# Dale-M/opendht

Measured on AMD Instinct MI355X. Metric: queries/sec, k=8 XOR-NN over 16M 160-bit IDs; % HBM roofline at 1/2/4/8 GPUs, higher is better.
Workload: dtype u32; 1 GPU; cfg2 batched k-NN: 65536 targets x 16777216 ids (2^24), k=8; n_ids=16777216, n_targets=65536, k=8, algo=batch, route=broadcast, ids_per_gpu=16777216, targets_per_gpu=65536, parallelism=id-range shards x1, inflight=3

## Files before the change

### opendht_amd/__init__.py

```python
import ctypes
import os

import numpy as np

__all__ = ["Context", "DhtGpuError", "NONE", "MAX_K", "lib", "LIB_PATH", "id_words"]

LIB_PATH = os.environ.get("DHTGPU_LIB") or os.path.join(os.path.dirname(os.path.abspath(__file__)), "libdhtgpu.so")
NONE = 0xFFFFFFFF
MAX_K = 32
EINVAL, ENOMEM, EDEVICE, ENOIDS, EUNSORTED, ERANGE = -1, -2, -3, -4, -5, -6

_u8p = ctypes.POINTER(ctypes.c_uint8)
_u32p = ctypes.POINTER(ctypes.c_uint32)
_u64p = ctypes.POINTER(ctypes.c_uint64)
_vp = ctypes.c_void_p
_lib = None


class DhtGpuError(RuntimeError):
    def __init__(self, code, what=""):
        msg = _lib.dhtgpu_strerror(code).decode() if _lib is not None else str(code)
        super().__init__(f"libdhtgpu: {what}: {msg} ({code})")
        self.code = code

# ... 167 lines not shown
    def set_global_indices(self, on):
        _check(lib().dhtgpu_set_global_indices(self._h, int(bool(on))), "set_global_indices")

    def set_sub_handles(self, on):
        _check(lib().dhtgpu_set_sub_handles(self._h, int(bool(on))), "set_sub_handles")

    def sub_handles_active(self, q, k):
        return bool(lib().dhtgpu_sub_handles_active(self._h, q, k))

    def handles_to_indices_dev(self, handles_ptr, m, out_ptr, idx_base=0, stream=None):
        _check(lib().dhtgpu_handles_to_indices_dev(self._h, handles_ptr, m, out_ptr, idx_base, stream),
               "handles_to_indices_dev")

    def select_prefix_dev(self, planes_ptr, stride, n, pbits, pval, out_planes_ptr, out_stride, out_gidx_ptr=None,
                          stream=None):
        cnt = ctypes.c_uint64()
        _check(lib().dhtgpu_select_prefix_dev(self._h, planes_ptr, stride, n, pbits, pval, out_planes_ptr, out_stride,
                                              out_gidx_ptr, ctypes.byref(cnt), stream), "select_prefix_dev")
        return cnt.value

    @property
    def num_ids(self):
        return int(lib().dhtgpu_num_ids(self._h))

    def get_ids(self, first=0, n=None):
        if n is None:
            n = self.num_ids - first
        out = np.empty((n, 20), dtype=np.uint8)
        _check(lib().dhtgpu_get_ids(self._h, first, n, _p(out, _u8p)), "get_ids")
        return out

    def ids_dev(self):
        p, s = _vp(), ctypes.c_uint64()
        _check(lib().dhtgpu_ids_dev(self._h, ctypes.byref(p), ctypes.byref(s)), "ids_dev")
        return p.value, s.value

    def topk(self, targets, k=8):
        t = _ids(targets, "targets")
        q = t.shape[0]
        out = np.empty((q, k), dtype=np.uint32)
        cnt = np.empty(q, dtype=np.uint32)
        _check(lib().dhtgpu_topk(self._h, _p(t, _u8p), q, k, _p(out, _u32p), _p(cnt, _u32p)), "topk")
        return out, cnt

    def index_topk(self, targets, k=8):
        t = _ids(targets, "targets")
        q = t.shape[0]
        out = np.empty((q, k), dtype=np.uint32)
        cnt = np.empty(q, dtype=np.uint32)
        _check(lib().dhtgpu_index_topk(self._h, _p(t, _u8p), q, k, _p(out, _u32p), _p(cnt, _u32p)), "index_topk")
        return out, cnt

    def index_build(self, stream=None):
        _check(lib().dhtgpu_index_build(self._h, stream), "index_build")

    def index_build_timed(self, stream=None):
        ms = (ctypes.c_float * 4)()
        _check(lib().dhtgpu_index_build_timed(self._h, stream, ms), "index_build_timed")
        return tuple(ms)

    def index_topk_dev(self, t_planes_ptr, t_stride, q, k, out_idx_ptr=None, out_cnt_ptr=None, out_rec_ptr=None,
                       idx_base=0, stream=None):
        _check(lib().dhtgpu_index_topk_dev(self._h, t_planes_ptr, t_stride, q, k, out_idx_ptr, out_cnt_ptr,
                                           out_rec_ptr, idx_base, stream), "index_topk_dev")

    def batch_topk(self, targets, k=8):
        t = _ids(targets, "targets")
        q = t.shape[0]
        out = np.empty((q, k), dtype=np.uint32)
        cnt = np.empty(q, dtype=np.uint32)
        _check(lib().dhtgpu_batch_topk(self._h, _p(t, _u8p), q, k, _p(out, _u32p), _p(cnt, _u32p)), "batch_topk")
        return out, cnt

    def batch_topk_dev(self, t_planes_ptr, t_stride, q, k, out_idx_ptr=None, out_cnt_ptr=None, out_rec_ptr=None,
                       idx_base=0, stream=None):
        _check(lib().dhtgpu_batch_topk_dev(self._h, t_planes_ptr, t_stride, q, k, out_idx_ptr, out_cnt_ptr,
                                           out_rec_ptr, idx_base, stream), "batch_topk_dev")

    def batch_topk_timed(self, t_planes_ptr, t_stride, q, k, out_idx_ptr, out_cnt_ptr, stream=None):
        ms = (ctypes.c_float * 4)()
        st = (ctypes.c_uint32 * 4)()
        _check(lib().dhtgpu_batch_topk_timed(self._h, t_planes_ptr, t_stride, q, k, out_idx_ptr, out_cnt_ptr,
                                             stream, ms, st), "batch_topk_timed")
        return tuple(ms), int(st[0]), int(st[1]), int(st[2])

    def batch_events(self, events):
        arr = (_vp * 8)(*[e.cuda_event for e in events])
        _check(lib().dhtgpu_batch_events(self._h, arr), "batch_events")

    def tie_words_dev(self, rec_ptr, q, k, idx_base, ties_ptr, tie_cap, row_base, out_words_ptr, stream=None):
        _check(lib().dhtgpu_tie_words_dev(self._h, rec_ptr, q, k, idx_base, ties_ptr, tie_cap, row_base,
                                          out_words_ptr, stream), "tie_words_dev")

    def topk_dev(self, t_planes_ptr, t_stride, q, k, out_idx_ptr=None, out_cnt_ptr=None, out_rec_ptr=None,
                 idx_base=0, stream=None):
        _check(lib().dhtgpu_topk_dev(self._h, t_planes_ptr, t_stride, q, k, out_idx_ptr, out_cnt_ptr,
                                     out_rec_ptr, idx_base, stream), "topk_dev")

    def find_closest(self, firsts, bucket_off, node_ids, good, targets, count=8):
        firsts = _ids(firsts, "firsts") if len(firsts) else np.zeros((0, 20), np.uint8)
        off = np.ascontiguousarray(bucket_off, dtype=np.uint32)
        nodes = _ids(node_ids, "node_ids") if len(node_ids) else np.zeros((1, 20), np.uint8)
        good = np.ascontiguousarray(good, dtype=np.uint8) if len(good) else np.zeros(1, np.uint8)
        t = _ids(targets, "targets")
        q = t.shape[0]
        out = np.empty((q, count), dtype=np.uint32)
        cnt = np.empty(q, dtype=np.uint32)
        _check(lib().dhtgpu_find_closest(self._h, firsts.shape[0], _p(firsts, _u8p), _p(off, _u32p),
                                         _p(nodes, _u8p), _p(good, _u8p), _p(t, _u8p), q, count,
                                         _p(out, _u32p), _p(cnt, _u32p)), "find_closest")
        return out, cnt

    def buffer_nodes(self, node_tail, af, targets, cand):
        t = _ids(targets, "targets")
        q = t.shape[0]
        cand = np.ascontiguousarray(cand, dtype=np.uint32).reshape(q, -1)
        alen = 4 if af == 4 else 16
        tail = np.ascontiguousarray(node_tail, dtype=np.uint8).reshape(-1, alen + 2)
        rec = 20 + alen + 2
        out = np.zeros((q, 8 * rec), dtype=np.uint8)
        ln = np.zeros(q, dtype=np.uint32)
        _check(lib().dhtgpu_buffer_nodes(self._h, _p(tail, _u8p), af, _p(t, _u8p), q, _p(cand, _u32p),
                                         cand.shape[1], _p(out, _u8p), _p(ln, _u32p)), "buffer_nodes")
        return out, ln

    def deserialize_nodes(self, af, myid, blobs, from_af, from_addr):
        alen = 4 if af == 4 else 16
        m = len(blobs)
        off = np.zeros(m + 1, dtype=np.uint64)
        for i, b in enumerate(blobs):
            off[i + 1] = off[i] + len(b)
        blob = np.frombuffer(b"".join(bytes(b) for b in blobs) or b"\0", dtype=np.uint8).copy()
        fa = np.ascontiguousarray(from_af, dtype=np.uint8).reshape(m) if m else np.zeros(1, np.uint8)
        fad = np.ascontiguousarray(from_addr, dtype=np.uint8).reshape(m, 16) if m else np.zeros((1, 16), np.uint8)
        cap = max(1, int(off[-1]) // (20 + alen + 2))
        ids = np.zeros((cap, 20), np.uint8)
        tail = np.zeros((cap, alen + 2), np.uint8)
        st = np.zeros(cap, np.uint8)
        ms = np.zeros(max(m, 1), np.uint8)
        nrec = ctypes.c_uint32()
        my = np.ascontiguousarray(myid, dtype=np.uint8).reshape(20)
        _check(lib().dhtgpu_deserialize_nodes(self._h, af, _p(my, _u8p), _p(blob, _u8p), _p(off, _u64p), m,
                                              _p(fa, _u8p), _p(fad, _u8p), _p(ids, _u8p), _p(tail, _u8p),
                                              _p(st, _u8p), _p(ms, _u8p), ctypes.byref(nrec)), "deserialize_nodes")
        r = nrec.value
        return ids[:r], tail[:r], st[:r], ms[:m]

    def net_prepare(self, dead=None, table_seed=0x5EED):
        d = None
        if dead is not None:
            d = np.ascontiguousarray(dead, dtype=np.uint8)
            if d.shape[0] != self.num_ids:
                raise ValueError("dead mask must have one byte per id")
        _check(lib().dhtgpu_net_prepare(self._h, _p(d, _u8p) if d is not None else None, table_seed), "net_prepare")

    def set_search_alpha(self, alpha):
        _check(lib().dhtgpu_set_search_alpha(self._h, int(alpha)), "set_search_alpha")
        self._alpha = int(alpha)

    def search_batch(self, targets, searchers, max_rounds=64, alpha=None):
        t = _ids(targets, "targets")
        q = t.shape[0]
        sr = np.ascontiguousarray(searchers, dtype=np.uint32).reshape(q)
        idx = np.empty((q, 64), np.uint32)
        fl = np.empty((q, 64), np.uint8)
        ln, rd, qs = (np.empty(q, np.uint32) for _ in range(3))
# ... 119 lines not shown
```

### opendht_amd/csrc/batch.hip

```cpp
#include "scan_dev.h"
#include <hip/hip_ext.h>

#include <mutex>

#include <algorithm>
#include <cmath>
#include <cstdlib>
#include <cstdio>
#include <string>
#include <vector>

namespace dhtgpu {
namespace {

constexpr int kF1Threads = 256;
constexpr int kF3Threads = 256;
constexpr uint32_t kF3Cap = 4096;
constexpr uint32_t kF3Per = kF3Cap / kF3Threads;
constexpr uint32_t kMaxLm = 19;
constexpr uint32_t kMaxSubBits = 11;
constexpr uint32_t kMaxQ = 1u << 22;
constexpr uint32_t kTieSlots = 8;
constexpr uint32_t kSets = 8;
constexpr uint32_t kCtrStride = 64;
// ... 648 lines not shown
                const uint32_t j0 = sb + tid4;
                const uint32_t v4[4] = {ring[r].x, ring[r].y, ring[r].z, ring[r].w};
                const uint32_t rem = hi - sb;
                uint32_t bw[4];
#pragma unroll
                for (uint32_t f = 0; f < 4; ++f) bw[f] = bm[__builtin_amdgcn_ubfe(v4[f], pre_off + 5, lm5) - wbase];
                bool sv[4];
                uint64_t bal[4], any = 0;
#pragma unroll
                for (uint32_t f = 0; f < 4; ++f) {
                    const uint32_t pre = __builtin_amdgcn_ubfe(v4[f], pre_off, a.Lm);
                    sv[f] = __builtin_amdgcn_ubfe(bw[f], pre, 1) != 0 && tid4 + f < rem;
                    bal[f] = __builtin_amdgcn_ballot_w64(sv[f]);
                    any |= bal[f];
                }
                if (any) {
                    const uint32_t l0 = (uint32_t)__ffsll((long long)any) - 1, l1 = 63u - (uint32_t)__clzll(any);
                    const uint32_t mylo = sv[0] ? v4[0] : sv[1] ? v4[1] : sv[2] ? v4[2] : v4[3];
                    const uint32_t myhi = sv[3] ? v4[3] : sv[2] ? v4[2] : sv[1] ? v4[1] : v4[0];
                    const uint32_t plo = top_bits((uint32_t)__builtin_amdgcn_readlane((int)mylo, (int)l0), a.b1);
                    const uint32_t phi = top_bits((uint32_t)__builtin_amdgcn_readlane((int)myhi, (int)l1), a.b1);
                    for (uint32_t p = plo; p <= phi; ++p) {
                        uint64_t bp[4];
                        uint32_t tot = 0;
#pragma unroll
                        for (uint32_t f = 0; f < 4; ++f) {
                            bp[f] = plo == phi ? bal[f] : bal[f] & __builtin_amdgcn_ballot_w64(top_bits(v4[f], a.b1) == p);
                            tot += (uint32_t)__popcll(bp[f]);
                        }
                        if (!tot) continue;
                        const uint32_t pl = p - p_first;
                        const bool glob = (p == p_first && sh_first) || (p == p_last && sh_last) || pl >= kDirParts;
                        uint32_t base = 0;
                        if (lane == 0) base = glob ? atomicAdd(pc + p, tot) : atomicAdd(cnt + pl, tot);
                        uint32_t pos = __builtin_amdgcn_readfirstlane(base);
#pragma unroll
                        for (uint32_t f = 0; f < 4; ++f) {
                            if ((bp[f] >> lane) & 1ull) {
                                const uint32_t at = __builtin_amdgcn_mbcnt_hi(
                                    (uint32_t)(bp[f] >> 32), __builtin_amdgcn_mbcnt_lo((uint32_t)bp[f], pos));
                                if (at < a.pcap) pb[(uint64_t)p * a.pcap + at] = make_uint2(v4[f], j0 + f);
                            }
                            pos += (uint32_t)__popcll(bp[f]);
                        }
                    }
                }
            }
            ring[r] = f2_load1<NT>(rs, lo, sb + kF2Ring * kF2Sub, lim);
        }
    }
    sync_lds();
    F2_STAMP(2);
    const uint32_t nown = min(p_last - p_first + 1u, kDirParts);
    for (uint32_t i = threadIdx.x; i < nown; i += kF2Threads) {
        const uint32_t p = p_first + i;
        if (!((p == p_first && sh_first) || (p == p_last && sh_last))) pc[p] = cnt[i];
    }
    (void)misc;
    F2_STAMP(5);
}

__device__ __forceinline__ bool id_less(uint32_t da, uint32_t ia, uint32_t db, uint32_t ib,
                                        const uint32_t* __restrict__ planes, uint64_t stride, const uint32_t* t) {
    if (da != db) return da < db;
    if (ia == ib) return false;
    uint32_t wa[DHT_W], wb[DHT_W];
    load_id(planes, stride, ia, wa);
    load_id(planes, stride, ib, wb);
    return xor_less_from(wa, ia, wb, ib, t, 1);
}

__device__ __forceinline__ uint32_t map_out(uint32_t x, const uint32_t* __restrict__ gidx, uint32_t base) {
    return gidx ? gidx[x] : x + base;
}


__device__ __forceinline__ void load_target(const uint32_t* __restrict__ tp, uint64_t ts, uint32_t qi, uint32_t* t) {
#pragma unroll
    for (int j = 0; j < DHT_W; ++j) t[j] = __builtin_amdgcn_readfirstlane(tp[(uint64_t)j * ts + qi]);
}

constexpr uint32_t kLaneMax = 256;

__host__ __device__ inline uint32_t f3_words(uint32_t nsub) {
    return (nsub + 1 + 17 + kF3Threads + 1 + 2 + 1) & ~1u;
}

struct RecOut {
    uint32_t* out;
    const uint32_t* planes;
    uint64_t stride;
    const uint32_t* gidx;
    uint32_t base;
    uint32_t w0_direct;
    uint32_t w0_shift, w0_pre;
};

__device__ __forceinline__ void rec_place(const RecOut& o, const uint32_t* __restrict__ planes, const uint32_t* gidx,
                                          uint32_t base, uint32_t k, uint32_t qi, uint32_t r, uint32_t x, uint32_t w0,
                                          bool w0_ok, uint32_t w1) {
    uint32_t* ro = o.out + ((uint64_t)qi * k + r) * 3;
    if (x == DHT_NONE) {
        ro[0] = DHT_NONE;
        ro[1] = DHT_NONE;
        ro[2] = DHT_NONE;
        return;
    }
    const uint32_t cl = gidx ? gidx[x] : x + base;
    ro[0] = w0_ok ? w0 : planes[x];
    ro[1] = w1;
    ro[2] = o.gidx ? o.gidx[cl] : cl + o.base;
}

struct F3Args {
    const uint2* pbuf; uint32_t* pcount; uint32_t pcap;
    const uint2* tbuf; uint32_t* tcount; uint32_t tcap;
    const uint32_t* tspill;
    uint32_t Lm, b1, Lq;
    uint32_t* bitmap; uint32_t nwords;
    const uint32_t* planes; uint64_t stride; uint64_t n;
    const uint32_t* tp; uint64_t ts; uint32_t k;
    const uint32_t* gidx; uint32_t base;
    uint32_t* out_idx; uint32_t* out_cnt;
    uint32_t* ctr; uint32_t* fb_list;
    uint8_t* fb_sub;
    uint32_t* pstat;
    uint4* tie_hdr;
    uint2* tie_cand;
    uint32_t* tie_cnt;
    const SubDesc* subs; uint32_t np_sub;
    uint32_t dbg;
    unsigned long long* stamps;
    uint32_t cap;
    RecOut rec;
    uint32_t Lmin;
    uint32_t nsets;
};

__device__ __forceinline__ void level_range(const uint32_t* sofs, uint32_t sq, uint32_t Lq, uint32_t Lmin, uint32_t want,
                                            uint32_t& lo, uint32_t& hi) {
    uint32_t L = Lq + 1;
    do {
        --L;
        const uint32_t sh_l = Lq - L;
        lo = sofs[(sq >> sh_l) << sh_l];
        hi = sofs[((sq >> sh_l) + 1) << sh_l];
    } while (hi - lo < want && L > Lmin);
}

__device__ __forceinline__ bool key2_less(uint32_t da, uint32_t a1, uint32_t ia, uint32_t db, uint32_t b1, uint32_t ib,
                                          const uint32_t* __restrict__ planes, uint64_t stride, const uint32_t* t) {
    if (da != db) return da < db;
    if (a1 != b1) return a1 < b1;
    return id_less(da, ia, db, ib, planes, stride, t);
}

__device__ __forceinline__ uint32_t wave_rank64(uint32_t md, uint32_t m1, uint32_t mm, uint32_t lane, bool* tie) {
    uint32_t rank = 0, eq = 0;
    for (uint32_t o = 0; o < mm; ++o) {
        const uint32_t xd = (uint32_t)__builtin_amdgcn_readlane((int)md, (int)o);
        const uint32_t x1 = (uint32_t)__builtin_amdgcn_readlane((int)m1, (int)o);
        rank += (uint32_t)(xd < md) | ((uint32_t)(xd == md) & (uint32_t)(x1 < m1));
        eq |= (uint32_t)(xd == md) & (uint32_t)(x1 == m1) & (uint32_t)(o != lane);
    }
    *tie = eq != 0;
    return rank;
}

// ... 26 lines not shown
}

__device__ void wave_rank_answer(const F3Args& a, uint2 me, uint32_t mm, uint32_t qi, uint32_t t0, uint32_t want,
                                 uint32_t lane) {
    const uint32_t w1 = a.planes[a.stride + (lane < mm ? me.y : 0u)];
    uint32_t t[DHT_W];
    load_target(a.tp, a.ts, qi, t);
    wave_rank_loaded(a, me, mm, qi, t0, want, lane, w1, t);
}

__device__ void f3_wave_answer(const F3Args& a, const uint2* S, uint32_t lo, uint32_t hi, uint32_t qi,
                               uint32_t t0, uint32_t want, uint32_t lane) {
    const uint32_t mm = hi - lo;
    if (mm <= 64) {
        wave_rank_answer(a, S[lo + (lane < mm ? lane : 0u)], mm, qi, t0, want, lane);
        return;
    }
    uint32_t t[DHT_W];
    load_target(a.tp, a.ts, qi, t);
    uint32_t* orow = a.out_idx + (uint64_t)qi * a.k;
    {
        uint32_t ed = DHT_NONE, e1 = DHT_NONE, ei = DHT_NONE, cnt = 0;
        for (uint32_t c = lo; c < hi; c += 64) {
            const bool v = c + lane < hi;
            const uint2 x = v ? S[c + lane] : make_uint2(0u, DHT_NONE);
            const uint32_t xd = x.x ^ t0, xi = x.y;
            const uint32_t x1 = v ? a.planes[a.stride + xi] ^ t[1] : DHT_NONE;
            uint32_t wd = cnt == want ? __builtin_amdgcn_readlane((int)ed, want - 1) : DHT_NONE;
            uint32_t w1 = cnt == want ? __builtin_amdgcn_readlane((int)e1, want - 1) : DHT_NONE;
            uint32_t wi = cnt == want ? __builtin_amdgcn_readlane((int)ei, want - 1) : DHT_NONE;
            uint64_t cm = __ballot(v && (cnt < want || key2_less(xd, x1, xi, wd, w1, wi, a.planes, a.stride, t)));
            while (cm) {
                const uint32_t l = (uint32_t)__ffsll((long long)cm) - 1;
                cm &= cm - 1;
                const uint32_t cd = __builtin_amdgcn_readlane((int)xd, l), c1 = __builtin_amdgcn_readlane((int)x1, l);
                const uint32_t ci = __builtin_amdgcn_readlane((int)xi, l);
                if (cnt == want && !key2_less(cd, c1, ci, wd, w1, wi, a.planes, a.stride, t)) continue;
                const bool closer = lane < cnt && key2_less(ed, e1, ei, cd, c1, ci, a.planes, a.stride, t);
                const uint32_t pos = (uint32_t)__popcll(__ballot(closer));
                const uint32_t ud = __shfl_up(ed, 1), u1 = __shfl_up(e1, 1), ui = __shfl_up(ei, 1);
                if (lane == pos) { ed = cd; e1 = c1; ei = ci; }
                else if (lane > pos) { ed = ud; e1 = u1; ei = ui; }
                cnt = cnt + 1 < want ? cnt + 1 : want;
                wd = cnt == want ? __builtin_amdgcn_readlane((int)ed, want - 1) : DHT_NONE;
                w1 = cnt == want ? __builtin_amdgcn_readlane((int)e1, want - 1) : DHT_NONE;
                wi = cnt == want ? __builtin_amdgcn_readlane((int)ei, want - 1) : DHT_NONE;
            }
        }
        if (a.rec.out) {
            if (lane < a.k)
                rec_place(a.rec, a.planes, a.gidx, a.base, a.k, qi, lane, lane < want ? ei : DHT_NONE, ed ^ t0,
                          a.rec.w0_direct, e1 ^ t[1]);
            return;
        }
        if (lane < want) orow[lane] = map_out(ei, a.gidx, a.base);
    }
    if (lane >= want && lane < a.k) orow[lane] = DHT_NONE;
    if (lane == 0) a.out_cnt[qi] = want;
}

template <int K, int CTRL>
__device__ __forceinline__ void f3_merge(uint32_t (&key)[K], uint32_t& lmin) {
    uint32_t b[K];
#pragma unroll
    for (int r = 0; r < K; ++r) b[r] = (uint32_t)__builtin_amdgcn_mov_dpp((int)key[K - 1 - r], CTRL, 0xF, 0xF, true);
    lmin = min(lmin, (uint32_t)__builtin_amdgcn_mov_dpp((int)lmin, CTRL, 0xF, 0xF, true));
#pragma unroll
    for (int r = 0; r < K; ++r) {
        lmin = min(lmin, max(key[r], b[r]));
        key[r] = min(key[r], b[r]);
    }
#pragma unroll
    for (int d = K / 2; d >= 1; d >>= 1) {
#pragma unroll
        for (int r = 0; r < K; ++r) {
            if (r & d) continue;
            const uint32_t x = min(key[r], key[r + d]), y = max(key[r], key[r + d]);
            key[r] = x;
            key[r + d] = y;
        }
    }
}

#define F3_STAMP(i) \
    do { if (Diag && (a.dbg & 256) && threadIdx.x == 0) a.stamps[(uint64_t)blockIdx.x * 16 + (i)] = __builtin_amdgcn_s_memrealtime(); } while (0)

template <int K, bool Diag, bool Exact, bool Subs>
__global__ __launch_bounds__(kF3Threads) void k_f3_answer(F3Args a) {
    extern __shared__ uint32_t sh[];
    const uint32_t p = blockIdx.x, np = gridDim.x;
    const uint32_t sub = p / a.np_sub, pl = p - sub * a.np_sub;
    if (Subs && a.np_sub != np) {
        const SubDesc d = a.subs[sub];
        a.planes = d.planes;
        a.stride = d.stride;
        a.gidx = d.gidx;
        a.base = d.base;
    }
    F3_STAMP(0);
    const uint32_t nsub = 1u << (a.Lq - a.b1);
    uint32_t* sofs = sh;
    uint32_t* wsum = sofs + nsub + 1;
    uint32_t* slow = wsum + 17;
    uint32_t* ntie = slow + kF3Threads + 1;
    uint2* S = reinterpret_cast<uint2*>(sh + f3_words(nsub));
    uint2* T = S + a.cap;
    for (uint32_t i = pl + a.np_sub * threadIdx.x; i < a.nwords; i += a.np_sub * kF3Threads)
        a.bitmap[sub * a.nwords + i] = 0;
    for (uint32_t i = threadIdx.x; i <= nsub; i += kF3Threads) sofs[i] = 0;
    if (threadIdx.x == 0) ntie[0] = ntie[1] = 0;
    static_assert(kF3Cap / kSets == 2 * kF3Threads && kF3Per == 2 * kSets, "gather layout");
    uint32_t ms[kSets];
#pragma unroll
    for (uint32_t x = 0; x < kSets; ++x) ms[x] = a.pcount[x * np + p];
    const uint32_t mt0 = a.tcount[p * kCtrStride];
    const uint2* tsrc = a.tbuf + (uint64_t)p * a.tcap;
    const uint2 tfirst = tsrc[threadIdx.x < a.tcap ? threadIdx.x : 0u];
    uint2 e[kF3Per];
    const uint2* pb = a.pbuf + (uint64_t)p * a.nsets * a.pcap;
#pragma unroll
    for (uint32_t u = 0; u < kF3Per; ++u) e[u] = make_uint2(0u, 0u);
    const uint32_t mt = mt0 < a.tcap ? mt0 : a.tcap;
    if (p == 0) {
        const uint32_t nsp = a.ctr[kSpill];
        if (nsp) {
            if (threadIdx.x == 0) ntie[2] = atomicAdd(a.ctr, nsp);
            sync_lds();
            for (uint32_t j = threadIdx.x; j < nsp; j += kF3Threads) {
                a.fb_list[ntie[2] + j] = a.tspill[j];
                a.fb_sub[ntie[2] + j] = 255;
            }
        }
    }
    sync_lds();
    uint32_t soff[kSets + 1];
    bool over = false;
    soff[0] = 0;
#pragma unroll
    for (uint32_t x = 0; x < kSets; ++x) {
        over = over || ms[x] > a.pcap;
        soff[x + 1] = soff[x] + (ms[x] < a.pcap ? ms[x] : a.pcap);
    }
    const uint32_t m = soff[kSets];
    if (threadIdx.x < kSets) a.pcount[threadIdx.x * np + p] = 0;
    if (threadIdx.x == 0) {
        a.pstat[p] = m;
        a.tcount[p * kCtrStride] = 0;
        if (p == 0) a.ctr[kSpill] = 0;
    }
    if (mt == 0) return;
    F3_STAMP(1);
    const uint32_t lane = lane_id(), wv = threadIdx.x >> 6;
    constexpr uint32_t NWV = kF3Threads / 64;
    if (m > a.cap || over) {
        if (threadIdx.x == 0) ntie[2] = atomicAdd(a.ctr, mt);
        sync_lds();
        for (uint32_t j = threadIdx.x; j < mt; j += kF3Threads) {
            a.fb_list[ntie[2] + j] = tsrc[j].y;
            a.fb_sub[ntie[2] + j] = (uint8_t)sub;
        }
        return;
    }
    const uint32_t smask = nsub - 1u;
    uint32_t rk[kF3Per];
    const uint32_t sq_sh = 32 - a.Lq;
    uint32_t valid = 0;
    {
#pragma unroll
        for (uint32_t u = 0; u < kF3Per; ++u) {
            const uint32_t j = u * kF3Threads + threadIdx.x;
            uint32_t x = 0, base = 0;
#pragma unroll
            for (uint32_t y = 1; y < kSets; ++y)
                if (j >= soff[y]) { x = y; base = soff[y]; }
            if (j < m) e[u] = pb[x * a.pcap + j - base];
            valid |= (uint32_t)(j < m) << u;
        }
    }
#pragma unroll
    for (uint32_t u = 0; u < kF3Per; ++u) {
        rk[u] = DHT_NONE;
        if ((valid >> u) & 1u) rk[u] = atomicAdd(sofs + __builtin_amdgcn_ubfe(e[u].x, sq_sh, a.Lq - a.b1), 1u);
    }
    sync_lds();
    F3_STAMP(2);
    scan_lds<kF3Threads>(sofs, nsub, wsum);
    if (threadIdx.x == 0) sofs[nsub] = m;
    sync_lds();
#pragma unroll
    for (uint32_t u = 0; u < kF3Per; ++u)
        if (rk[u] != DHT_NONE) S[sofs[__builtin_amdgcn_ubfe(e[u].x, sq_sh, a.Lq - a.b1)] + rk[u]] = e[u];
    F3_STAMP(3);
    const uint32_t want = Exact ? (uint32_t)K : (a.n < a.k ? (uint32_t)a.n : a.k);
    const bool full_row = Exact && ((uintptr_t)a.out_idx & 15) == 0;
    for (uint32_t t0i = 0; t0i < mt; t0i += kF3Threads) {
        const uint32_t mtr = mt - t0i < kF3Threads ? mt - t0i : kF3Threads;
        if (threadIdx.x < mtr) T[threadIdx.x] = t0i ? tsrc[t0i + threadIdx.x] : tfirst;
        if (threadIdx.x == 0) slow[kF3Threads] = 0;
        sync_lds();
        if (t0i == 0) F3_STAMP(4);
        const uint32_t G = a.Lmin >= 12 ? (mtr <= kF3Threads / 4 ? 4u : mtr <= kF3Threads / 2 ? 2u : 1u) : 1u;
        const uint32_t slot = G == 4 ? threadIdx.x >> 2 : G == 2 ? threadIdx.x >> 1 : lane * NWV + wv;
        const uint32_t gj = threadIdx.x & (G - 1);
        uint32_t tq = 0, tt0 = 0, tlo = 0, thi = 0;
        bool tinl = false;
        if (slot < mtr) {
            const uint2 te = T[slot];
            const uint32_t t0 = te.x, qi = te.y;
            uint32_t lo = 0, hi = 0;
            level_range(sofs, top_bits(t0, a.Lq) & smask, a.Lq, a.Lmin, want, lo, hi);
            const uint32_t mm = hi - lo;
            if (t0i == 0) F3_STAMP(8);
            if (mm < want) {
                if (gj == 0) {
                    const uint32_t at = atomicAdd(a.ctr, 1u);
                    a.fb_list[at] = qi;
                    a.fb_sub[at] = (uint8_t)sub;
                }
            } else if (mm > kLaneMax || a.Lm == 0) {
                if (gj == 0) {
                    slow[atomicAdd(slow + kF3Threads, 1u)] = slot;
                    atomicAdd(ntie + 1, 1u);
                }
            } else {
                uint32_t dk[K], ok[K];
                uint32_t rmin = DHT_NONE;
                if (a.Lmin >= 12) {
                    uint32_t key[K];
#pragma unroll
                    for (int r = 0; r < K; ++r) key[r] = DHT_NONE;
                    uint32_t lmin = DHT_NONE;
                    uint32_t o = lo + gj;
                    uint32_t nxt = S[o < hi ? o : lo].x;
                    for (; o < hi; o += G) {
                        const uint32_t c = ((nxt ^ t0) << 12) | o;
                        nxt = S[o + G < hi ? o + G : o].x;
                        lmin = min(lmin, max(c, key[K - 1]));
#pragma unroll
                        for (int r = K - 1; r > 0; --r) key[r] = med3_u32(key[r - 1], key[r], c);
                        key[0] = min(key[0], c);
                    }
                    if (t0i == 0) F3_STAMP(9);
                    if (G >= 2) f3_merge<K, 0xB1>(key, lmin);
                    if (G == 4) f3_merge<K, 0x4E>(key, lmin);
#pragma unroll
                    for (int r = 0; r < K; ++r) {
                        dk[r] = key[r] == DHT_NONE ? DHT_NONE : key[r] >> 12;
                        ok[r] = key[r] & 0xFFFu;
                    }
                    rmin = lmin == DHT_NONE ? DHT_NONE : lmin >> 12;
                } else {
#pragma unroll
                    for (int r = 0; r < K; ++r) { dk[r] = DHT_NONE; ok[r] = DHT_NONE; }
                    uint32_t nxt = S[lo].x;
                    for (uint32_t o = lo; o < hi; ++o) {
                        const uint32_t d = nxt ^ t0;
                        nxt = S[o + 1 < hi ? o + 1 : o].x;
                        const bool ins = d < dk[K - 1];
                        rmin = min(rmin, ins ? dk[K - 1] : d);
                        if (ins) {
#pragma unroll
                            for (int r = K - 1; r > 0; --r) {
                                const bool up = d < dk[r - 1];
                                const bool here = d < dk[r];
                                ok[r] = up ? ok[r - 1] : (here ? o : ok[r]);
                                dk[r] = up ? dk[r - 1] : (here ? d : dk[r]);
                            }
                            if (d < dk[0]) { dk[0] = d; ok[0] = o; }
                        }
                    }
                }
                if (t0i == 0) F3_STAMP(10);
                bool tie = rmin == dk[want - 1];
#pragma unroll
                for (int r = 0; r + 1 < K; ++r) tie = tie || ((uint32_t)r + 1 <= want && dk[r] == dk[r + 1]);
                if (tie && !Subs) {
                    if (gj == 0) {
                        tinl = true;
                        tq = qi;
                        tt0 = t0;
                        tlo = lo;
                        thi = hi;
                        atomicAdd(ntie + 1, 1u);
                    }
                } else if (tie) {
                    uint32_t tsl = kTieSlots;
                    {
                        const uint64_t want_slot = __ballot(gj == 0 && mm <= 64), leaders = __ballot(gj == 0);
                        const uint32_t first = (uint32_t)__ffsll((long long)leaders) - 1;
                        uint32_t base = 0;
                        if (lane == first) {
                            atomicAdd(ntie + 1, (uint32_t)__popcll(leaders));
                            if (want_slot) base = atomicAdd(ntie, (uint32_t)__popcll(want_slot));
                        }
                        base = (uint32_t)__builtin_amdgcn_readlane((int)base, (int)first);
                        const uint32_t leader = lane & ~(G - 1);
                        if (mm <= 64) tsl = base + (uint32_t)__popcll(want_slot & ((1ull << leader) - 1ull));
                    }
                    if (tsl < kTieSlots) {
                        const uint32_t g = p * kTieSlots + tsl;
                        uint2* dst = a.tie_cand + (uint64_t)g * 64;
                        for (uint32_t o = gj; o < mm; o += G) dst[o] = S[lo + o];
                        if (gj == 0) a.tie_hdr[g] = make_uint4(qi, t0, mm, 0u);
                    } else if (gj == 0) {
                        slow[atomicAdd(slow + kF3Threads, 1u)] = slot;
                    }
                } else if (gj == 0 || (K == 8 && a.rec.out && full_row && G > 1 && ((uintptr_t)a.rec.out & 15) == 0)) {
                    uint32_t* orow = a.out_idx + (uint64_t)qi * a.k;
                    uint32_t res[K];
                    if (a.rec.out) {
                        uint32_t w0[K], w1[K], gi[K];
#pragma unroll
                        for (int r = 0; r < K; ++r) {
                            const uint2 e = S[(uint32_t)r < want && ok[r] < a.cap ? ok[r] : 0u];
                            res[r] = e.y;
                            w0[r] = e.x;
                        }
#pragma unroll
                        for (int r = 0; r < K; ++r) {
                            if (!a.rec.w0_direct)
                                w0[r] = a.rec.w0_shift ? ((a.rec.w0_pre | (Subs ? sub : 0u)) << (32 - a.rec.w0_shift)) |
                                                             (w0[r] >> a.rec.w0_shift)
                                                       : a.planes[res[r]];
                            w1[r] = a.planes[a.stride + res[r]];
                            res[r] = map_out(res[r], a.gidx, a.base);
                        }
#pragma unroll
                        for (int r = 0; r < K; ++r) gi[r] = a.rec.gidx ? a.rec.gidx[res[r]] : res[r] + a.rec.base;
                        uint32_t* ro = a.rec.out + (uint64_t)qi * a.k * 3;
                        if (full_row && ((uintptr_t)a.rec.out & 15) == 0) {
                            uint32_t wds[3 * K];
#pragma unroll
                            for (int r = 0; r < K; ++r) {
                                wds[3 * r] = w0[r];
                                wds[3 * r + 1] = w1[r];
                                wds[3 * r + 2] = gi[r];
                            }
                            if (K == 8 && G > 1) {
                                auto put = [&](uint32_t c, uint32_t c_lo, uint32_t c_hi) {
                                    uint32_t x[4];
#pragma unroll
                                    for (int i = 0; i < 4; ++i) {
                                        x[i] = 0u;
#pragma unroll
                                        for (uint32_t cc = 0; cc < 6; ++cc)
                                            if (cc >= c_lo && cc < c_hi) x[i] = c == cc ? wds[(4 * cc + i) % (3 * K)] : x[i];
                                    }
                                    *reinterpret_cast<uint4*>(ro + 4 * c) = make_uint4(x[0], x[1], x[2], x[3]);
                                };
                                put(gj, 0u, 4u);
                                if (gj + G < 6) put(gj + G, 2u, 6u);
                                if (gj + 2 * G < 6) put(gj + 2 * G, 4u, 6u);
                            } else {
#pragma unroll
                                for (int r = 0; r < 3 * K; r += 4)
                                    *reinterpret_cast<uint4*>(ro + r) = make_uint4(wds[r], wds[r + 1], wds[r + 2], wds[r + 3]);
                            }
                        } else {
#pragma unroll
                            for (int r = 0; r < K; ++r) {
// ... 16 lines not shown
                        }
#pragma unroll
                        for (int r = 0; r < K; r += 4)
                            *reinterpret_cast<uint4*>(orow + r) = make_uint4(res[r], res[r + 1], res[r + 2], res[r + 3]);
                        a.out_cnt[qi] = want;
                    } else {
#pragma unroll
                        for (int r = 0; r < K; ++r) res[r] = (uint32_t)r < want ? S[ok[r] < a.cap ? ok[r] : 0u].y : 0u;
                        if (a.gidx) {
#pragma unroll
                            for (int r = 0; r < K; ++r) res[r] = a.gidx[res[r]];
                        } else {
#pragma unroll
                            for (int r = 0; r < K; ++r) res[r] += a.base;
                        }
#pragma unroll
                        for (int r = 0; r < K; ++r)
                            if ((uint32_t)r < a.k) orow[r] = (uint32_t)r < want ? res[r] : DHT_NONE;
                        a.out_cnt[qi] = want;
                    }
                }
            }
        }
        if (!Subs) {
            uint64_t tb = __ballot(tinl);
            while (tb) {
                const int L0 = __ffsll((long long)tb) - 1;
                tb &= tb - 1;
                const uint32_t lo0 = (uint32_t)__builtin_amdgcn_readlane((int)tlo, L0);
                const uint32_t mm0 = (uint32_t)__builtin_amdgcn_readlane((int)thi, L0) - lo0;
                const uint32_t q0 = (uint32_t)__builtin_amdgcn_readlane((int)tq, L0);
                const uint32_t t00 = (uint32_t)__builtin_amdgcn_readlane((int)tt0, L0);
                if (mm0 > 64 || !tb) {
                    f3_wave_answer(a, S, lo0, lo0 + mm0, q0, t00, want, lane);
                    continue;
                }
                const int L1 = __ffsll((long long)tb) - 1;
                const uint32_t lo1 = (uint32_t)__builtin_amdgcn_readlane((int)tlo, L1);
                const uint32_t mm1 = (uint32_t)__builtin_amdgcn_readlane((int)thi, L1) - lo1;
                if (mm1 > 64) {
                    f3_wave_answer(a, S, lo0, lo0 + mm0, q0, t00, want, lane);
                    continue;
                }
                tb &= tb - 1;
                const uint32_t q1 = (uint32_t)__builtin_amdgcn_readlane((int)tq, L1);
                const uint32_t t01 = (uint32_t)__builtin_amdgcn_readlane((int)tt0, L1);
                const uint2 c0 = S[lo0 + (lane < mm0 ? lane : 0u)], c1 = S[lo1 + (lane < mm1 ? lane : 0u)];
                const uint32_t w10 = a.planes[a.stride + (lane < mm0 ? c0.y : 0u)];
                const uint32_t w11 = a.planes[a.stride + (lane < mm1 ? c1.y : 0u)];
                uint32_t tw0[DHT_W], tw1[DHT_W];
                load_target(a.tp, a.ts, q0, tw0);
                load_target(a.tp, a.ts, q1, tw1);
                wave_rank_loaded(a, c0, mm0, q0, t00, want, lane, w10, tw0);
                wave_rank_loaded(a, c1, mm1, q1, t01, want, lane, w11, tw1);
            }
        }
        if (Diag && (a.dbg & 256) && t0i == 0) {
            if (lane == 0) a.stamps[2ull * 8192 * 16 + (uint64_t)blockIdx.x * 16 + wv] = __builtin_amdgcn_s_memrealtime();
        }
        sync_lds();
        if (t0i == 0) F3_STAMP(5);
        if (Diag && (a.dbg & 256) && threadIdx.x == 0 && t0i == 0) {
            a.stamps[(uint64_t)blockIdx.x * 16 + 11] = __builtin_amdgcn_s_memrealtime();
            a.stamps[(uint64_t)blockIdx.x * 16 + 13] = mt;
            a.stamps[(uint64_t)blockIdx.x * 16 + 12] =
                (__builtin_amdgcn_s_getreg((31 << 11) | 4) >> 8 & 0xFFu) | (__builtin_amdgcn_s_getreg((31 << 11) | 20) & 0xFu) << 8;
            a.stamps[(uint64_t)blockIdx.x * 16 + 14] = ntie[0];
        }
        const uint32_t ns = slow[kF3Threads];
        for (uint32_t i = wv; i < ns; i += NWV) {
            const uint2 te = T[slow[i]];
            const uint32_t t0 = __builtin_amdgcn_readfirstlane(te.x);
            const uint32_t qi = __builtin_amdgcn_readfirstlane(te.y);
            uint32_t lo = 0, hi = 0;
            level_range(sofs, top_bits(t0, a.Lq) & smask, a.Lq, a.Lmin, want, lo, hi);
            f3_wave_answer(a, S, __builtin_amdgcn_readfirstlane(lo), __builtin_amdgcn_readfirstlane(hi), qi, t0, want,
                           lane);
        }
        if (ns || t0i + kF3Threads < mt) sync_lds();
        if (t0i == 0) F3_STAMP(6);
    }
    sync_lds();
    if (threadIdx.x == 0 && ntie[1]) atomicAdd(a.ctr + 2, ntie[1]);
    if (threadIdx.x == 0 && ntie[0]) a.tie_cnt[p] = ntie[0] < kTieSlots ? ntie[0] : kTieSlots;
    F3_STAMP(7);
}

constexpr uint32_t kF4Threads = scan::WAVES * 64;
constexpr uint32_t kFbGroup = scan::WAVES * kScanTargets;
constexpr uint32_t kFbBlocks = 256;
constexpr uint32_t kFbCands = 256;
constexpr uint32_t kFbSingle = 64;

struct FbArgs {
    uint32_t* rec;
    uint32_t* done;
    uint32_t nfb;
    uint32_t np_ties;
    uint32_t* hint;
};

__device__ __forceinline__ uint32_t ld_sc1(const uint32_t* p) {
    return __hip_atomic_load(p, __ATOMIC_RELAXED, __HIP_MEMORY_SCOPE_AGENT);
}

__device__ __forceinline__ uint32_t wave_min_u32(uint32_t x) {
#pragma unroll
    for (int o = 32; o >= 1; o >>= 1) x = min(x, (uint32_t)__shfl_xor((int)x, o));
    return x;
}

__device__ void fb_merge(const F3Args& a, const FbArgs& f, uint32_t g, uint32_t S, uint32_t cnt, uint32_t* lds,
                         uint32_t gsize = kFbGroup) {
    const uint32_t lane = lane_id(), wv = threadIdx.x >> 6;
    const uint32_t k = a.k, nt = cnt - g * gsize < gsize ? cnt - g * gsize : gsize;
    uint32_t* buf = lds + wv * 2 * kFbCands;
    for (uint32_t j = wv; j < nt; j += scan::WAVES) {
        const uint32_t qr = __builtin_amdgcn_readfirstlane(a.fb_list[g * gsize + j]);
        uint32_t t[DHT_W];
        load_target(a.tp, a.ts, qr, t);
        for (uint32_t c = lane; c < S * k; c += 64) {
            const uint32_t l = c / k, r = c - l * k;
            const uint32_t* src = f.rec + ((((uint64_t)g * S + l) * kFbGroup + j) * k + r) * 6;
            const uint32_t w0 = ld_sc1(src), ix = ld_sc1(src + 5);
            buf[2 * c] = ix == DHT_NONE ? DHT_NONE : w0 ^ t[0];
            buf[2 * c + 1] = ix;
        }
        __builtin_amdgcn_fence(__ATOMIC_RELEASE, "wavefront");
        __builtin_amdgcn_wave_barrier();
        __builtin_amdgcn_fence(__ATOMIC_ACQUIRE, "wavefront");
        uint32_t p = 0, hd = DHT_NONE, hi = DHT_NONE;
        if (lane < S) {
            hd = buf[2 * lane * k];
            hi = buf[2 * lane * k + 1];
        }
        uint32_t* orow = a.out_idx + (uint64_t)qr * k;
        uint32_t r = 0;
        for (; r < k; ++r) {
            const bool valid = hi != DHT_NONE;
            const uint32_t m = wave_min_u32(valid ? hd : DHT_NONE);
            const uint64_t cand = __ballot(valid && hd == m);
            if (!cand) break;
            uint32_t win = (uint32_t)__ffsll((long long)cand) - 1;
            if (__popcll(cand) > 1) {
                uint64_t rest = cand & (cand - 1);
                while (rest) {
                    const uint32_t l2 = (uint32_t)__ffsll((long long)rest) - 1;
                    rest &= rest - 1;
                    const uint32_t ib = __builtin_amdgcn_readlane((int)hi, (int)win);
                    const uint32_t i2 = __builtin_amdgcn_readlane((int)hi, (int)l2);
                    if (id_less(m, i2, m, ib, a.planes, a.stride, t)) win = l2;
                }
            }
            const uint32_t wi = __builtin_amdgcn_readlane((int)hi, (int)win);
            if (lane == 0) {
                if (a.rec.out)
                    rec_place(a.rec, a.planes, a.gidx, a.base, k, qr, r, wi, m ^ t[0], true, a.planes[a.stride + wi]);
                else
                    orow[r] = map_out(wi, a.gidx, a.base);
            }
            if (lane == win) {
                ++p;
                hd = p < k ? buf[2 * (lane * k + p)] : DHT_NONE;
                hi = p < k ? buf[2 * (lane * k + p) + 1] : DHT_NONE;
            }
        }
// ... 1339 lines not shown
```

Measured before the change: 2.065 billion queries/s.

## Resolve first-word XOR ties in-block via LDS twin hash table

Adds an LDS hash table built during the F3 answer kernel that detects candidate IDs sharing the same first 32-bit word (twins). It records up to 16 such candidates with their second word, so tied top-k rows in the first target batch can be resolved inline instead of being sent to the slower tie/fallback path. This adds atomicCAS hashing work, extra global loads and LDS header space to every block, and only applies in restricted cases (no subs, no record output, first tile).

```diff
diff --git a/opendht_amd/__init__.py b/opendht_amd/__init__.py
--- a/opendht_amd/__init__.py
+++ b/opendht_amd/__init__.py
@@ -273,6 +273,7 @@
         st = (ctypes.c_uint32 * 4)()
         _check(lib().dhtgpu_batch_topk_timed(self._h, t_planes_ptr, t_stride, q, k, out_idx_ptr, out_cnt_ptr,
                                              stream, ms, st), "batch_topk_timed")
+        self.last_batch_stats = tuple(int(x) for x in st)
         return tuple(ms), int(st[0]), int(st[1]), int(st[2])
 
     def batch_events(self, events):
diff --git a/opendht_amd/csrc/batch.hip b/opendht_amd/csrc/batch.hip
--- a/opendht_amd/csrc/batch.hip
+++ b/opendht_amd/csrc/batch.hip
@@ -754,8 +754,22 @@
 
 constexpr uint32_t kLaneMax = 256;
 
+constexpr uint32_t kTwinProbes = 16;
+constexpr uint32_t kTwinCap = 16;
+constexpr uint32_t kTwinWords = 8;
+constexpr uint32_t kTwinMul0 = 0x9E3779B1u, kTwinMul1 = 0x85EBCA6Bu;
+constexpr uint32_t kTwinMinTable = 512;
+constexpr uint32_t kTwinHdr = 4 + kTwinWords + 3 * kTwinCap;
+
+__device__ __forceinline__ uint32_t twin_slot(uint32_t w, uint32_t r, uint32_t tsz, uint32_t hsh) {
+    uint32_t s = (w * kTwinMul0) >> hsh;
+    s = s >= tsz ? s - tsz : s;
+    s += r * ((((w * kTwinMul1) >> 30) << 1) | 1u);
+    return s >= tsz ? s - tsz : s;
+}
+
 __host__ __device__ inline uint32_t f3_words(uint32_t nsub) {
-    return (nsub + 1 + 17 + kF3Threads + 1 + 2 + 1) & ~1u;
+    return (nsub + 1 + 17 + kF3Threads + 1 + 2 + 1 + kTwinHdr + 3) & ~3u;
 }
 
 struct RecOut {
@@ -948,6 +962,56 @@
     }
 }
 
+template <int K>
+__device__ __forceinline__ bool f3_twin_row(const F3Args& a, const uint2* S, const uint32_t (&dk)[K],
+                                            const uint32_t (&ok)[K], uint32_t rmin, uint32_t want, uint32_t t0,
+                                            uint32_t tw1, uint32_t qi, uint32_t nl, const uint32_t* tl0,
+                                            const uint32_t* tli, const uint32_t* tl1) {
+    nl = nl < kTwinCap ? nl : kTwinCap;
+    uint32_t mask = 0, d = 0;
+    bool good = true;
+#pragma unroll
+    for (int r = 0; r < K; ++r) {
+        bool tied = (uint32_t)r + 1 == want && rmin == dk[r];
+        if (r > 0) tied = tied || dk[r - 1] == dk[r];
+        if (r + 1 < K) tied = tied || dk[r + 1] == dk[r];
+        if (!tied || (uint32_t)r >= want) continue;
+        if (!mask) d = dk[r];
+        good = good && dk[r] == d;
+        mask |= 1u << r;
+    }
+    const uint32_t w = d ^ t0, r0 = (uint32_t)__ffs((int)mask) - 1u, cin = (uint32_t)__popc(mask);
+    uint32_t nm = 0;
+    for (uint32_t i = 0; i < nl; ++i) {
+        if (tl0[i] != w) continue;
+        ++nm;
+        for (uint32_t o = 0; o < i; ++o) good = good && !(tl0[o] == w && tl1[o] == tl1[i]);
+    }
+    if (!good || !mask || nm < 2 || nm < cin) return false;
+    uint32_t* orow = a.out_idx + (uint64_t)qi * a.k;
+    for (uint32_t i = 0; i < nl; ++i) {
+        if (tl0[i] != w) continue;
+        const uint32_t di = tl1[i] ^ tw1;
+        uint32_t c = 0;
+        for (uint32_t o = 0; o < nl; ++o) c += (uint32_t)(tl0[o] == w && (tl1[o] ^ tw1) < di);
+        if (c < cin) orow[r0 + c] = map_out(tli[i], a.gidx, a.base);
+    }
+#pragma unroll
+    for (int r = 0; r < K; ++r) {
+        if ((uint32_t)r >= a.k || ((mask >> r) & 1u)) continue;
+        orow[r] = (uint32_t)r < want ? map_out(S[ok[r] < a.cap ? ok[r] : 0u].y, a.gidx, a.base) : DHT_NONE;
+    }
+    a.out_cnt[qi] = want;
+    return true;
+}
+
+__device__ __forceinline__ uint32_t f3_pick_word(const uint2 (&e)[kF3Per], uint32_t u) {
+    uint32_t w = 0;
+#pragma unroll
+    for (uint32_t x = 0; x < kF3Per; ++x) w |= e[x].x & (0u - (uint32_t)(u == x));
+    return w;
+}
+
 #define F3_STAMP(i) \
     do { if (Diag && (a.dbg & 256) && threadIdx.x == 0) a.stamps[(uint64_t)blockIdx.x * 16 + (i)] = __builtin_amdgcn_s_memrealtime(); } while (0)
 
@@ -971,10 +1035,21 @@
     uint32_t* ntie = slow + kF3Threads + 1;
     uint2* S = reinterpret_cast<uint2*>(sh + f3_words(nsub));
     uint2* T = S + a.cap;
+    uint32_t* twh = ntie + 3;
+    uint32_t* tww = twh + 4;
+    uint32_t* tl0 = tww + kTwinWords;
+    uint32_t* tli = tl0 + kTwinCap;
+    uint32_t* tl1 = tli + kTwinCap;
+    uint32_t* twt = reinterpret_cast<uint32_t*>(S);
+    const uint32_t tsz = 2u * a.cap < 8192u ? 2u * a.cap : 8192u;
+    const uint32_t thsh = (uint32_t)__clz((int)(tsz - 1u));
+    const bool twins = !Subs && K <= 16 && !a.rec.out && a.b1 != 0 && tsz >= kTwinMinTable;
+    const uint32_t tw_none = ~(pl << (32 - (a.b1 ? a.b1 : 1u)));
     for (uint32_t i = pl + a.np_sub * threadIdx.x; i < a.nwords; i += a.np_sub * kF3Threads)
         a.bitmap[sub * a.nwords + i] = 0;
     for (uint32_t i = threadIdx.x; i <= nsub; i += kF3Threads) sofs[i] = 0;
     if (threadIdx.x == 0) ntie[0] = ntie[1] = 0;
+    if (threadIdx.x < 4) twh[threadIdx.x] = 0;
     static_assert(kF3Cap / kSets == 2 * kF3Threads && kF3Per == 2 * kSets, "gather layout");
     uint32_t ms[kSets];
 #pragma unroll
@@ -998,6 +1073,11 @@
             }
         }
     }
+    if (twins) {
+        for (uint32_t i = threadIdx.x * 4; i < tsz; i += kF3Threads * 4)
+            *reinterpret_cast<uint4*>(twt + i) = make_uint4(tw_none, tw_none, tw_none, tw_none);
+        T[threadIdx.x] = tfirst;
+    }
     sync_lds();
     uint32_t soff[kSets + 1];
     bool over = false;
@@ -1018,6 +1098,10 @@
     F3_STAMP(1);
     const uint32_t lane = lane_id(), wv = threadIdx.x >> 6;
     constexpr uint32_t NWV = kF3Threads / 64;
+    auto group_of = [&](uint32_t mtr) {
+        return a.Lmin >= 12 ? (mtr <= kF3Threads / 4 ? 4u : mtr <= kF3Threads / 2 ? 2u : 1u) : 1u;
+    };
+    auto slot_of = [&](uint32_t G) { return G == 4 ? threadIdx.x >> 2 : G == 2 ? threadIdx.x >> 1 : lane * NWV + wv; };
     if (m > a.cap || over) {
         if (threadIdx.x == 0) ntie[2] = atomicAdd(a.ctr, mt);
         sync_lds();
@@ -1043,6 +1127,45 @@
             valid |= (uint32_t)(j < m) << u;
         }
     }
+    uint32_t tw1 = 0;
+    if (twins) {
+        const uint32_t mtr = mt < kF3Threads ? mt : kF3Threads, s0 = slot_of(group_of(mtr));
+        if (s0 < mtr) tw1 = a.tp[a.ts + T[s0].y];
+    }
+    uint32_t tw_at = DHT_NONE, tw_w1 = 0;
+    if (twins) {
+        uint32_t pend = 0, met = 0;
+        bool bad = false;
+#pragma unroll
+        for (uint32_t u = 0; u < kF3Per; ++u) {
+            if (!((valid >> u) & 1u)) continue;
+            const uint32_t w = e[u].x, old = atomicCAS(twt + twin_slot(w, 0, tsz, thsh), tw_none, w);
+            bad = bad || w == tw_none;
+            met |= (uint32_t)(old == w) << u;
+            pend |= (uint32_t)(old != w && old != tw_none) << u;
+        }
+        uint32_t r = 1;
+#pragma nounroll
+        while (pend) {
+            const uint32_t u = (uint32_t)__ffs((int)pend) - 1u, w = f3_pick_word(e, u);
+            const uint32_t old = atomicCAS(twt + twin_slot(w, r, tsz, thsh), tw_none, w);
+            if (old == w) met |= 1u << u;
+            ++r;
+            if (old == w || old == tw_none || r == kTwinProbes) {
+                bad = bad || (old != w && old != tw_none);
+                pend &= pend - 1u;
+                r = 1;
+            }
+        }
+#pragma nounroll
+        while (met) {
+            const uint32_t u = (uint32_t)__ffs((int)met) - 1u, at = atomicAdd(twh, 1u);
+            met &= met - 1u;
+            if (at < kTwinWords) tww[at] = f3_pick_word(e, u);
+            else bad = true;
+        }
+        if (bad) twh[2] = 1;
+    }
 #pragma unroll
     for (uint32_t u = 0; u < kF3Per; ++u) {
         rk[u] = DHT_NONE;
@@ -1050,6 +1173,40 @@
     }
     sync_lds();
     F3_STAMP(2);
+    if (twins && twh[0]) {
+        const uint32_t nw = twh[0] < kTwinWords ? twh[0] : kTwinWords;
+#pragma nounroll
+        for (uint32_t i = 0; i < nw; ++i) {
+            const uint32_t w = tww[i];
+            bool dup = false;
+            for (uint32_t j = 0; j < i; ++j) dup = dup || tww[j] == w;
+            uint32_t hm = 0;
+#pragma unroll
+            for (uint32_t u = 0; u < kF3Per; ++u) hm |= (uint32_t)(((valid >> u) & 1u) && e[u].x == w) << u;
+            if (dup) hm = 0;
+#pragma nounroll
+            while (hm) {
+                const uint32_t u = (uint32_t)__ffs((int)hm) - 1u, at = atomicAdd(twh + 1, 1u);
+                hm &= hm - 1u;
+                if (at >= kTwinCap) {
+                    twh[2] = 1;
+                    continue;
+                }
+                uint32_t idx = 0;
+#pragma unroll
+                for (uint32_t x = 0; x < kF3Per; ++x) idx |= e[x].y & (0u - (uint32_t)(u == x));
+                tl0[at] = w;
+                tli[at] = idx;
+                const uint32_t w1 = a.planes[a.stride + idx];
+                if (tw_at == DHT_NONE) {
+                    tw_at = at;
+                    tw_w1 = w1;
+                } else {
+                    tl1[at] = w1;
+                }
+            }
+        }
+    }
     scan_lds<kF3Threads>(sofs, nsub, wsum);
     if (threadIdx.x == 0) sofs[nsub] = m;
     sync_lds();
@@ -1063,10 +1220,11 @@
         const uint32_t mtr = mt - t0i < kF3Threads ? mt - t0i : kF3Threads;
         if (threadIdx.x < mtr) T[threadIdx.x] = t0i ? tsrc[t0i + threadIdx.x] : tfirst;
         if (threadIdx.x == 0) slow[kF3Threads] = 0;
+        if (t0i == 0 && tw_at != DHT_NONE) tl1[tw_at] = tw_w1;
         sync_lds();
         if (t0i == 0) F3_STAMP(4);
-        const uint32_t G = a.Lmin >= 12 ? (mtr <= kF3Threads / 4 ? 4u : mtr <= kF3Threads / 2 ? 2u : 1u) : 1u;
-        const uint32_t slot = G == 4 ? threadIdx.x >> 2 : G == 2 ? threadIdx.x >> 1 : lane * NWV + wv;
+        const uint32_t G = group_of(mtr);
+        const uint32_t slot = slot_of(G);
         const uint32_t gj = threadIdx.x & (G - 1);
         uint32_t tq = 0, tt0 = 0, tlo = 0, thi = 0;
         bool tinl = false;
@@ -1141,7 +1299,10 @@
 #pragma unroll
                 for (int r = 0; r + 1 < K; ++r) tie = tie || ((uint32_t)r + 1 <= want && dk[r] == dk[r + 1]);
                 if (tie && !Subs) {
-                    if (gj == 0) {
+                    if (gj == 0 && twins && t0i == 0 && twh[2] == 0 &&
+                        f3_twin_row<K>(a, S, dk, ok, rmin, want, t0, tw1, qi, twh[1], tl0, tli, tl1)) {
+                        atomicAdd(twh + 3, 1u);
+                    } else if (gj == 0) {
                         tinl = true;
                         tq = qi;
                         tt0 = t0;
@@ -1324,6 +1485,7 @@
     }
     sync_lds();
     if (threadIdx.x == 0 && ntie[1]) atomicAdd(a.ctr + 2, ntie[1]);
+    if (threadIdx.x == 0 && twh[3]) atomicAdd(a.ctr + 3, twh[3]);
     if (threadIdx.x == 0 && ntie[0]) a.tie_cnt[p] = ntie[0] < kTieSlots ? ntie[0] : kTieSlots;
     F3_STAMP(7);
 }
```

Result: slower. 1.514 billion queries/s (-26.7%).
